# fluhus/frackyfrac

Hardware: NVIDIA B200
Metric: UniFrac sample-pairs/sec (unweighted) (higher is better)
Workload: dtype u8 x u8 -> s32 (tcgen05 kind::i8, exact), s64 chunk / row sums, f32 ratio / output

## Files before the change

### frackyfrac_b200/csrc/frc_internal.h

```cpp
#pragma once
#include <cuda_runtime.h>
#include <cstdint>
#include <string>

namespace frc {

constexpr int kTile = 128;
constexpr int kKBlock = 64;

inline int64_t round_up(int64_t x, int64_t m) { return (x + m - 1) / m * m; }
inline int64_t tri(int64_t i) { return i * (i - 1) / 2; }

struct DevTree {
  int32_t n_nodes = 0;
  int32_t height = 0;
  const int32_t* parent = nullptr;
  const double* length = nullptr;
  const int32_t* child_ptr = nullptr;
  const int32_t* child_idx = nullptr;
  const int32_t* level_nodes = nullptr;
  const int32_t* level_parent = nullptr;
};

struct DevCsr {
  int64_t n_samples = 0;
  int64_t nnz = 0;
  const int64_t* row_ptr = nullptr;
  const int32_t* col = nullptr;
  const double* val = nullptr;
};

struct PeerPtrs {
  uint32_t* p[8] = {nullptr, nullptr, nullptr, nullptr, nullptr, nullptr, nullptr, nullptr};
  int n = 0;
  int self = 0;
};

struct Tile { int32_t ti, tj; };

struct Exceptions {
  unsigned long long* count = nullptr;
  int64_t* index = nullptr;
  double* value = nullptr;
  int32_t cap = 0;
};

int launch_embed_f64(const DevTree& t, const int32_t* level_ptr_host, const DevCsr& a, double* E,
                     int64_t ld, int64_t s_base, cudaStream_t s, int32_t* K = nullptr, int32_t kp = 0);
int launch_totals_f64(const double* E, int32_t n_nodes, int64_t ld, int64_t n_samples,
                      double* total, cudaStream_t s);
int launch_totals_fast_f64(const double* E, int32_t n_nodes, int64_t ld, const double* mult, double* total,
                           double* scratch, cudaStream_t s);
int launch_normalize_f64(double* E, int32_t n_nodes, int64_t ld, int64_t n_samples,
// ... 74 lines not shown
  const double* scale = nullptr;
  const int32_t* shift = nullptr;
  int32_t n = 0;
  bool biased = false;
};
TcOperands* tc_operands_create(const void* P, const void* Bh, const void* Bl, int64_t np, int32_t kp,
                               bool i8, const TcChunks& chunks, const double* len_col, const double* flag_u,
                               std::string* err);
TcOperands* tc_operands_create_bits(const uint32_t* bitsS, int64_t np, int32_t kp, const uint8_t* qa,
                                    const uint8_t* qh, const uint8_t* ql, const TcChunks& chunks,
                                    const double* len_col, const double* flag_u, const long long* r_int,
                                    double unit, std::string* err);
void tc_operands_set_int(TcOperands* o, const long long* r_int, double unit);
void tc_operands_destroy(TcOperands* o);
int tc_chunk_kblocks();
int launch_unweighted_tc(const TcOperands* ops, const double* r, const Tile* tiles, int32_t n_tiles,
                         int64_t n_samples, int64_t first, float* out, double flag_below,
                         uint32_t* flagged, unsigned long long* n_flagged, int num_sms, cudaStream_t s);
int launch_unweighted_fixup(const TcOperands* ops, const uint32_t* flagged,
                            const unsigned long long* n_flagged, unsigned long long* count_host,
                            int64_t first, float* out, const Exceptions& ex, int num_sms, cudaStream_t s);
bool tc_setup(std::string* err);

}
```

### frackyfrac_b200/csrc/job.cu

```cuda
#include <algorithm>
#include <atomic>
#include <chrono>
#include <climits>
#include <cmath>
#include <cstdio>
#include <cstdlib>
#include <cstring>
#include <functional>
#include <memory>
#include <string>
#include <thread>
#include <vector>

#if defined(__x86_64__)
#include <immintrin.h>
#endif

#include "../../include/frcfrc_cuda.h"
#include "frc_internal.h"
#include "host_pool.h"
#include "plan.h"

using namespace frc;
using frc_host::Pool;
// ... 60 lines not shown
constexpr int kMaxParts = 8;

struct Knobs {
  bool trace = false;
  int bands_per_rank = 0;
  int widen_threads = 0;
  int ws_slab = 0;
  bool uw_bf16 = false;
  bool u8_acc_f64 = false;
  bool feed_bits = false;
  bool embed_levels = false;
  int peer_push = -1;
  int group_binades = 3;
  int shard = -1;
  int capacity = -1;
  static Knobs read() {
    Knobs k;
    auto num = [](const char* name, int dflt) { const char* e = getenv(name); return e && *e ? atoi(e) : dflt; };
    auto is = [](const char* name, const char* v) { const char* e = getenv(name); return e && !strcmp(e, v); };
    k.trace = getenv("FRC_TRACE") != nullptr;
    k.bands_per_rank = std::max(0, num("FRC_BANDS", 0));
    k.widen_threads = std::max(0, num("FRC_WIDEN_THREADS", 0));
    k.ws_slab = std::max(0, num("FRC_WS_SLAB", 0));
    k.uw_bf16 = is("FRC_UW_KERNEL", "bf16");
    k.u8_acc_f64 = is("FRC_U8_ACC", "f64");
    k.feed_bits = is("FRC_UW_FEED", "bits");
    k.embed_levels = num("FRC_EMBED_LEVELS", 0) == 1;
    k.peer_push = num("FRC_PEER_PUSH", -1);
    k.group_binades = num("FRC_U8_GROUP_BINADES", 3);
    k.shard = num("FRC_SHARD", -1);
    k.capacity = num("FRC_CAPACITY", -1);
    return k;
  }
};

struct DeviceGuard {
  int prev = -1;
  DeviceGuard() { if (cudaGetDevice(&prev) != cudaSuccess) { prev = -1; cudaGetLastError(); } }
  ~DeviceGuard() { if (prev >= 0) cudaSetDevice(prev); }
};

}

struct DevCtx {
  int device = 0;
  int num_sms = 0;
// ... 68 lines not shown
namespace {

struct Part {
  frc_job* job = nullptr;
  const Shared* sh = nullptr;
  DevCtx* dc = nullptr;
  int index = 0;
  int owner = 0;
  int rc = FRC_OK;
  std::string err;
  frc_info_t info{};

  std::vector<int> mine;
  std::vector<Band> bands;
  std::vector<Tile> tiles;

  int32_t shard_w0 = 0, shard_nw = 0;
  int64_t csr_k0 = 0, csr_k1 = 0;
  PanelMap pm;
  struct CapGroup {
    int shard = 0;
    int64_t first = 0, count = 0;
    int32_t tile_off = 0;
    std::vector<int32_t> coff;
    float* out = nullptr;
    uint32_t* flagged = nullptr;
    unsigned long long* cnt = nullptr;
    unsigned long long* n_flagged_host = nullptr;
    Exceptions ex;
    cudaEvent_t done = nullptr;
// ... 11 lines not shown
  Tile* d_tiles = nullptr;
  int32_t* d_level_ptr = nullptr;
  int32_t* d_post = nullptr;
  unsigned long long* d_flag_counts = nullptr;
  int64_t ws_slab = 0;
  bool peer_push = false;
  uint32_t* d_bits2[2] = {nullptr, nullptr};
  PeerPtrs peers[2];
  int64_t run_count = 0;
  void *d_q0 = nullptr, *d_q1 = nullptr, *d_q2 = nullptr;
  int32_t *d_order = nullptr, *d_col_exp = nullptr;
  uint32_t* d_qam = nullptr;
  uint32_t* d_bitsS = nullptr;
  long long* d_r_int = nullptr;
  long long* d_fix_ws[2] = {nullptr, nullptr};
  uint8_t* d_need = nullptr;
  double *d_lenq = nullptr, *d_len_col = nullptr, *d_flag_u = nullptr, *d_qerr = nullptr;
  TcChunks d_chunks;
  float* d_lenf = nullptr;
  const double* d_mult = nullptr;
  double *d_E = nullptr, *d_total = nullptr, *d_W = nullptr, *d_r = nullptr, *d_scratch = nullptr;
  float* d_A = nullptr;
  int32_t* d_K = nullptr;
  uint32_t *d_bits = nullptr, *d_node_scratch = nullptr;
  void *d_P = nullptr, *d_Bh = nullptr, *d_Bl = nullptr;
  TcOperands* tc = nullptr;
  int64_t* d_list_ptr = nullptr;
  int32_t* d_list_id = nullptr;
  double* d_list_val = nullptr;
  int64_t list_cap = 0;
// ... 356 lines not shown
    else
      launches += launch_exact_pairs(p->d_E, p->dtree.length, sh.B, sh.np, sh.weighted, b.first, b.count, sl.dev64, s);
    PART_CUDA(p, cudaEventRecord(sl.k1, s));
  } else {
    unsigned long long* cnt = p->d_flag_counts + idx;
    *sl.ex.count = 0;
    if (sh.weighted) {
      launches += launch_weighted_tiles(p->pm, sh.np, sh.kp, p->d_lenf, sh.prescale, p->d_W, p->d_tiles + b.tile_off,
                                        b.n_tiles, sh.N, b.first, sl.dev32, kFlagBelowW, sl.flagged, cnt, dc->num_sms, s,
                                        p->d_K);
      PART_CUDA(p, cudaEventRecord(sl.k1, s));
      launches += launch_weighted_fixup(p->dcsr, p->dtree, sh.opts.normalize == 1 ? p->d_total : nullptr, p->d_W,
                                        sl.flagged, cnt, sl.n_flagged_host, b.first, p->d_fix_ws[si], kFixupCtas,
                                        sl.dev32, sl.ex, s, p->d_K, sh.kp);
    } else {
      launches += launch_unweighted_tc(p->tc, p->d_r, p->d_tiles + b.tile_off, b.n_tiles, sh.N, b.first, sl.dev32,
                                       kFlagBelow, sl.flagged, cnt, dc->num_sms, s);
      PART_CUDA(p, cudaEventRecord(sl.k1, s));
      launches += launch_unweighted_fixup(p->tc, sl.flagged, cnt, sl.n_flagged_host, b.first, sl.dev32, sl.ex,
                                          dc->num_sms, s);
    }
  }
  PART_CUDA(p, cudaGetLastError());
  PART_CUDA(p, cudaEventRecord(sl.k2, s));
  if (sh.d2h) {
    cudaStream_t cs = dc->stream[2];
    PART_CUDA(p, cudaStreamWaitEvent(cs, sl.k2, 0));
    if (sh.exact) {
      PART_CUDA(p, cudaMemcpyAsync(sl.host64, sl.dev64, sizeof(double) * b.count, cudaMemcpyDeviceToHost, cs));
      p->info.d2h_bytes += static_cast<int64_t>(sizeof(double)) * b.count;
    } else {
      PART_CUDA(p, cudaMemcpyAsync(sl.host32, sl.dev32, sizeof(float) * b.count, cudaMemcpyDeviceToHost, cs));
// ... 474 lines not shown
      p->max_band = std::max(p->max_band, sh.bands[k].count);
    }
  const bool fast_uw = !sh.exact && !sh.weighted;
  if (sh.capacity) {
    const std::vector<CapGroupPlan> groups =
        plan_capacity_groups(p->bands, sh.N, sh.shards.shard_rows, sh.shards.n_shards, p->tiles, p->band_group);
    for (const CapGroupPlan& gp : groups) {
      if (gp.count >= (1LL << 32)) return pfail(p, FRC_ERR_UNSUPPORTED, "capacity mode: a row shard holds 2^32 pairs or more");
      Part::CapGroup g;
      g.shard = gp.shard; g.first = gp.first; g.count = gp.count; g.tile_off = gp.tile_off; g.coff = gp.coff;
      p->cap.push_back(g);
    }
  } else if (!sh.exact) {
    for (Band& b : p->bands) append_band_tiles(b, fast_uw, p->tiles);
  }
  std::vector<uint8_t> need;
  if (fast_uw && sh.shards.ranges.size() > 1 && sh.fused_embed) need = operand_need_blocks(p->tiles, sh.np, true);
  const Range& own = sh.shards.ranges[p->owner][0];
  p->shard_w0 = static_cast<int32_t>(own.s0 / 32);
  p->shard_nw = static_cast<int32_t>((own.s1 - own.s0) / 32);
  p->csr_k0 = 0; p->csr_k1 = sh.nnz;
  if (sh.exchange != Shared::kNone && fast_uw && sh.N > 0) {
    const int64_t* rp = reinterpret_cast<const int64_t*>(sh.stage_in + sh.in_rowptr.off);
    p->csr_k0 = rp[std::min(sh.N, own.s0)]; p->csr_k1 = rp[std::min(sh.N, own.s1)];
  }
  SegAlloc seg;
  const Seg s_tiles = seg(sizeof(Tile) * p->tiles.size()), s_need = seg(need.size());
  char* st = pin_alloc<char>(p, seg.total);
  if (!st) return p->rc;
  char* d_small = dev_alloc<char>(p, seg.total);
  if (!d_small) return p->rc;
  if (!p->tiles.empty()) memcpy(st + s_tiles.off, p->tiles.data(), s_tiles.bytes);
  if (!need.empty()) memcpy(st + s_need.off, need.data(), s_need.bytes);
  if (!(p->d_plan = dev_alloc<char>(p, sh.plan_bytes))) return p->rc;
  if (!(p->d_in = dev_alloc<char>(p, sh.in_bytes))) return p->rc;
  for (cudaEvent_t* e : {&p->ev_h2d0, &p->ev_h2d1, &p->ev_embed0, &p->ev_embed1, &p->ev_run1})
    PART_CUDA(p, cudaEventCreate(e));
  for (cudaEvent_t* e : {&p->ev_join, &p->ev_bits, &p->ev_rsum, &p->ev_shard})
    PART_CUDA(p, cudaEventCreateWithFlags(e, cudaEventDisableTiming));
  cudaStream_t s0 = dc->stream[0];
  PART_CUDA(p, cudaEventRecord(p->ev_h2d0, s0));
  PART_CUDA(p, cudaMemcpyAsync(p->d_plan, sh.stage_plan, sh.plan_bytes, cudaMemcpyHostToDevice, s0));
  if (seg.total) PART_CUDA(p, cudaMemcpyAsync(d_small, st, seg.total, cudaMemcpyHostToDevice, s0));
  p->info.h2d_bytes = static_cast<int64_t>(sh.plan_bytes + seg.total);
  char* d = p->d_plan;
  char* di = p->d_in;
  p->dcsr.n_samples = sh.N; p->dcsr.nnz = sh.nnz;
  p->dcsr.row_ptr = reinterpret_cast<int64_t*>(di + sh.in_rowptr.off);
// ... 12 lines not shown
  p->d_mult = sh.node_mult ? reinterpret_cast<const double*>(di + sh.in_mult.off) : nullptr;
  p->d_q0 = d + sh.pl_q0.off;
  p->d_q1 = d + sh.pl_hi.off;
  p->d_q2 = d + sh.pl_lo.off;
  p->d_lenq = reinterpret_cast<double*>(d + sh.pl_lenq.off);
  p->d_order = reinterpret_cast<int32_t*>(d + sh.pl_order.off);
  p->d_col_exp = reinterpret_cast<int32_t*>(d + sh.pl_cexp.off);
  p->d_len_col = reinterpret_cast<double*>(d + sh.pl_lcol.off);
  p->d_chunks.end = reinterpret_cast<int32_t*>(d + sh.pl_cend.off);
  p->d_chunks.scale = reinterpret_cast<double*>(d + sh.pl_cscale.off);
  p->d_chunks.n = static_cast<int32_t>(sh.cols.chunk_end.size());
  p->d_chunks.shift = sh.cols.chunk_shift.empty() ? nullptr : reinterpret_cast<int32_t*>(d + sh.pl_cshift.off);
  p->d_chunks.biased = sh.cols.i8 && sh.cols.biased;
  p->d_tiles = reinterpret_cast<Tile*>(d_small + s_tiles.off);
  p->d_need = need.empty() ? nullptr : reinterpret_cast<uint8_t*>(d_small + s_need.off);

  const int chunks = weighted_scratch_chunks(B);
  const bool i8 = sh.cols.i8, intacc = sh.cols.intacc;
  if (sh.exact || sh.weighted) {
    const int64_t per = static_cast<int64_t>(p->shard_nw) * 32;
    p->ws_slab = sh.exact ? sh.np : std::min<int64_t>(per, std::max<int64_t>(kTile, (2LL << 30) / (8LL * B) / kTile * kTile));
    if (!sh.exact && sh.knobs.ws_slab > 0)
      p->ws_slab = std::min<int64_t>(per, round_up(sh.knobs.ws_slab, kTile));
    if (!(p->d_E = dev_alloc<double>(p, static_cast<size_t>(B) * p->ws_slab))) return p->rc;
    if (!(p->d_total = dev_alloc<double>(p, sh.np))) return p->rc;
    if (sh.unsorted_l && !(p->d_list_ptr = dev_alloc<int64_t>(p, sh.N + 2))) return p->rc;
    if (!sh.exact) {
      const size_t a_samples = sh.capacity ? static_cast<size_t>(2 * sh.shards.shard_rows) : static_cast<size_t>(sh.np);
      if (!(p->d_A = dev_alloc<float>(p, static_cast<size_t>(sh.kp) * a_samples))) return p->rc;
      if (sh.keyed && !(p->d_K = dev_alloc<int32_t>(p, static_cast<size_t>(sh.kp) * a_samples))) return p->rc;
// ... 62 lines not shown
    } else if (!(p->d_bits = dev_alloc<uint32_t>(p, std::max<size_t>(words, 64)))) return p->rc;
    const size_t ns = sh.fused_embed ? static_cast<size_t>(presence_node_scratch_words(B, p->shard_nw)) : 0;
    if (ns && !(p->d_node_scratch = dev_alloc<uint32_t>(p, ns))) return p->rc;
    const size_t opsz = sh.bits_feed ? 256 : static_cast<size_t>(sh.np) * sh.kp * (i8 ? 1 : 2);
    if (!(p->d_P = dev_alloc<char>(p, opsz))) return p->rc;
    if (!(p->d_Bh = dev_alloc<char>(p, opsz))) return p->rc;
    if (!(p->d_Bl = dev_alloc<char>(p, opsz))) return p->rc;
    if (sh.bits_feed && !(p->d_bitsS = dev_alloc<uint32_t>(p, static_cast<size_t>(sh.np) * (sh.kp / 32)))) return p->rc;
    if (!(p->d_r = dev_alloc<double>(p, sh.np))) return p->rc;
    if (!(p->d_scratch = dev_alloc<double>(p, static_cast<size_t>(chunks) * sh.np))) return p->rc;
    if (!(p->d_flag_counts = dev_alloc<unsigned long long>(p, p->mine.size() + 1))) return p->rc;
    if (i8 && !(p->d_flag_u = dev_alloc<double>(p, 1))) return p->rc;
    if (i8 && !(p->d_qerr = dev_alloc<double>(p, sh.kp))) return p->rc;
    if (i8 && !(p->d_qam = dev_alloc<uint32_t>(p, sh.kp))) return p->rc;
    if (intacc && !(p->d_r_int = dev_alloc<long long>(p, sh.np))) return p->rc;
    std::string terr;
    if (sh.bits_feed) {
      p->tc = tc_operands_create_bits(p->d_bitsS, sh.np, sh.kp, static_cast<const uint8_t*>(p->d_q0),
                                      static_cast<const uint8_t*>(p->d_q1), static_cast<const uint8_t*>(p->d_q2),
                                      p->d_chunks, p->d_len_col, p->d_flag_u, p->d_r_int,
                                      std::ldexp(1.0, sh.cols.e_min), &terr);
    } else {
      p->tc = tc_operands_create(p->d_P, p->d_Bh, p->d_Bl, sh.np, sh.kp, i8, p->d_chunks, p->d_len_col, p->d_flag_u, &terr);
      if (p->tc && intacc) tc_operands_set_int(p->tc, p->d_r_int, std::ldexp(1.0, sh.cols.e_min));
    }
    if (!p->tc) return pfail(p, FRC_ERR_CUDA, terr);
    if (i8) {
      p->info.kernel_launches += launch_quantize_lengths(
          p->d_len_col, p->d_col_exp, sh.kp, static_cast<uint8_t*>(p->d_q0), static_cast<uint8_t*>(p->d_q1),
          static_cast<uint8_t*>(p->d_q2), p->d_qam, p->d_lenq, p->d_qerr, p->d_flag_u, s0);
// ... 577 lines not shown
```

### frackyfrac_b200/csrc/plan.cpp

```cpp
#include "plan.h"

#include <algorithm>
#include <climits>
#include <cmath>
#include <cstring>

namespace frc {

static std::vector<int> band_owners_lpt(const std::vector<int64_t>& rows, int world) {
  const size_t n = rows.size() > 0 ? rows.size() - 1 : 0;
  std::vector<int> owner(n, 0);
  std::vector<size_t> order(n);
  std::vector<int64_t> cnt(n);
  for (size_t k = 0; k < n; ++k) {
    order[k] = k;
    cnt[k] = tri(rows[k + 1]) - (rows[k] >= 2 ? tri(rows[k]) : 0);
  }
  std::stable_sort(order.begin(), order.end(), [&](size_t a, size_t b) { return cnt[a] > cnt[b]; });
  std::vector<int64_t> load(world, 0);
  for (size_t k : order) {
    int best = 0;
    for (int r = 1; r < world; ++r)
      if (load[r] < load[best]) best = r;
    owner[k] = best;
// ... 256 lines not shown
    const int32_t rows_blk = std::min<int32_t>(9, t1 - t0 + 1);
    const int32_t cols_blk = std::max<int32_t>(1, 74 / rows_blk);
    for (int32_t tb = t0; tb <= t1; tb += rows_blk) {
      const int32_t te = std::min(t1, tb + rows_blk - 1);
      for (int32_t pb = 0; 2 * pb <= te; pb += cols_blk)
        for (int32_t tp = pb; tp < pb + cols_blk && 2 * tp <= te; ++tp)
          for (int32_t ti = std::max(2 * tp, tb); ti <= te; ++ti) tiles.push_back({ti, 2 * tp});
    }
  } else {
    for (int32_t tj = 0; tj <= t1; ++tj)
      for (int32_t ti = std::max(tj, t0); ti <= t1; ++ti) tiles.push_back({ti, tj});
  }
  b.n_tiles = static_cast<int32_t>(tiles.size()) - b.tile_off;
}

std::vector<uint8_t> operand_need_blocks(const std::vector<Tile>& tiles, int64_t np, bool pair_tiles) {
  std::vector<uint8_t> need(static_cast<size_t>((np + 255) / 256), 0);
  const int32_t pairw = pair_tiles ? 2 : 1;
  for (const Tile& t : tiles) {
    need[t.ti / 2] |= 2;
    for (int32_t c = 0; c < pairw; ++c)
      if ((static_cast<int64_t>(t.tj) + c) * kTile < np) need[(t.tj + c) / 2] |= 1;
  }
  return need;
}

bool check_preorder(const int32_t* parent, int32_t B, int32_t* depth, int32_t* bad_parent, int32_t* bad_order) {
  *bad_parent = 0; *bad_order = 0;
  std::vector<int32_t> on_path(B + 1, 0);
  depth[0] = 0;
// ... 138 lines not shown
    for (int c = 0; c <= sp.n_shards; ++c) out_coff[k * (sp.n_shards + 1) + c] = g[k].coff[c];
  }
  for (size_t k = 0; k < tiles.size(); ++k) { out_tiles[2 * k] = tiles[k].ti; out_tiles[2 * k + 1] = tiles[k].tj; }
  return static_cast<int64_t>(g.size());
}

int64_t frc_debug_band_tiles(int64_t row0, int64_t row1, int32_t pair_tiles, int32_t* out2, int64_t cap) {
  frc::Band b;
  b.row0 = row0; b.row1 = row1;
  std::vector<frc::Tile> tiles;
  frc::append_band_tiles(b, pair_tiles != 0, tiles);
  for (size_t k = 0; k < tiles.size() && static_cast<int64_t>(k) < cap; ++k) { out2[2 * k] = tiles[k].ti; out2[2 * k + 1] = tiles[k].tj; }
  return static_cast<int64_t>(tiles.size());
}

int32_t frc_debug_plan_columns(const double* length, int32_t n_nodes, int32_t want_i8, int32_t group_binades,
                               int32_t force_f64, int32_t* col_order, int32_t* col_exp, double* len_col, int32_t cap,
                               int32_t* chunk_end, double* chunk_scale, int32_t* chunk_shift, int32_t* info) {
  const frc::ColumnPlan p = frc::plan_columns(length, n_nodes, want_i8 != 0, group_binades, force_f64 != 0, 64);
  if (p.kp > cap || p.chunk_end.size() > 64) return -p.kp;
  for (int32_t k = 0; k < p.kp; ++k) {
    col_order[k] = p.col_order[k];
    col_exp[k] = p.col_exp.empty() ? 0 : p.col_exp[k];
    len_col[k] = p.len_col[k];
  }
  for (size_t c = 0; c < p.chunk_end.size(); ++c) {
    chunk_end[c] = p.chunk_end[c];
    chunk_scale[c] = p.chunk_scale[c];
    chunk_shift[c] = p.chunk_shift.empty() ? 0 : p.chunk_shift[c];
  }
// ... 28 lines not shown
```

### frackyfrac_b200/csrc/plan.h

```cpp
#pragma once
#include <cstdint>
#include <string>
#include <vector>

#include "frc_internal.h"

namespace frc {

struct Band {
  int64_t row0 = 0, row1 = 0;
  int64_t first = 0, count = 0;
  int32_t tile_off = 0, n_tiles = 0;
  int owner = 0;
};

std::vector<int64_t> band_boundaries(int64_t N, int64_t requested, int world, bool d2h, int per_rank, int value_bytes);
std::vector<int> band_owners(const std::vector<int64_t>& rows, int world);
std::vector<Band> make_bands(int64_t N, int64_t requested, int world, bool d2h, int per_rank, int value_bytes);

struct Range { int64_t s0, s1, slot; };
struct ShardPlan {
  enum Mode { kWhole, kSharded, kCapacity };
  int64_t np = 0, shard_rows = 0;
  int n_shards = 1;
// ... 18 lines not shown
  bool intacc = false;
  bool biased = false;
  int32_t kp = 0;
  int32_t e_min = 0;
  std::vector<int32_t> col_order;
  std::vector<int32_t> col_exp;
  std::vector<double> len_col;
  std::vector<int32_t> chunk_end;
  std::vector<double> chunk_scale;
  std::vector<int32_t> chunk_shift;
};
ColumnPlan plan_columns(const double* length, int32_t n_nodes, bool want_i8, int group_binades, bool force_f64_acc,
                        int bf16_chunk_kblocks);

void append_band_tiles(Band& b, bool pair_tiles, std::vector<Tile>& tiles);
std::vector<uint8_t> operand_need_blocks(const std::vector<Tile>& tiles, int64_t np, bool pair_tiles);

struct TreeLevels {
  int32_t height = -1;
  int32_t bad_parent = 0, bad_order = 0;
  std::vector<int32_t> level_ptr;
};
bool check_preorder(const int32_t* parent, int32_t n_nodes, int32_t* depth, int32_t* bad_parent, int32_t* bad_order);
TreeLevels tree_levels(const int32_t* parent, int32_t n_nodes, int32_t* level_nodes, int32_t* level_parent);
bool tree_children(const int32_t* parent, int32_t n_nodes, int32_t* child_ptr, int32_t* child_idx);
void tree_post_order(const int32_t* parent, int32_t n_nodes, int32_t* post_order);

struct PrunedTree {
  int32_t n_nodes = 0;
  std::vector<int32_t> parent, new_of_old;
// ... 7 lines not shown
```

### frackyfrac_b200/csrc/unweighted_tc.cu

```cuda
#include <cuda.h>
#include <cuda_runtime.h>

#include <cstdio>
#include <cstdlib>
#include <type_traits>

#include "frc_internal.h"
#include "ptx.cuh"
#include "wire.cuh"

namespace frc {

namespace {

constexpr int BM = 128, BN = 128, BK = 64, UK = 16;
constexpr int A_BYTES = BM * BK * 2;
constexpr int B_BYTES = BN * BK * 2;
constexpr int EPI_WARP0 = 2;
constexpr int DN = 2 * BN;
constexpr uint32_t TMEM_COLS = 2 * DN;

constexpr int STAGES2 = 6;
constexpr int STAGE2_BYTES = A_BYTES + B_BYTES;
constexpr int NUM_BARS2 = 2 * STAGES2 + 4;
// ... 57 lines not shown
#pragma unroll
    for (int x = 0; x < 8; ++x) {
      const int64_t i = i0 + n0 + x;
      if (i < n_samples && j < i) {
        out[off] = dv[x];
        if (fu[x]) {
          unsigned long long slot = atomicAdd(n_flagged, 1ULL);
          flagged[slot] = static_cast<uint32_t>(off);
        }
      }
      off += i;
    }
  }
}

template <int kMode>
__global__ void __cluster_dims__(2, 1, 1) __launch_bounds__(THREADS2, 1)
k_unweighted_tc2(const __grid_constant__ CUtensorMap mapP, const __grid_constant__ CUtensorMap mapBh,
                 const __grid_constant__ CUtensorMap mapBl, const int32_t* __restrict__ chunk_end,
                 const double* __restrict__ chunk_scale, const int32_t* __restrict__ chunk_shift,
                 int32_t n_chunks, int32_t biased, const double* __restrict__ r,
                 const long long* __restrict__ r_int, double unit, const Tile* __restrict__ tiles, int32_t n_tiles,
                 int64_t n_samples, int64_t first, float* __restrict__ out, double flag_below,
                 const double* __restrict__ flag_u_ptr, uint32_t* __restrict__ flagged,
                 unsigned long long* __restrict__ n_flagged, int dbg) {
  (void)dbg;
  constexpr bool kI8 = kMode != 0;
  constexpr bool kInt = kMode == 2;
  extern __shared__ uint8_t smem_raw[];
  const uint32_t raw = ptx::smem_u32(smem_raw);
  const uint32_t pad = ((raw + 1023u) & ~1023u) - raw;
  uint8_t* smem = smem_raw + pad;
  const uint32_t smem_base = raw + pad;
  const uint32_t bar_base = smem_base + STAGES2 * STAGE2_BYTES;
  auto full_bar = [&](int s) { return bar_base + 8u * s; };
  auto empty_bar = [&](int s) { return bar_base + 8u * (STAGES2 + s); };
  auto tfull_bar = [&](int b) { return bar_base + 8u * (2 * STAGES2 + b); };
  auto tempty_bar = [&](int b) { return bar_base + 8u * (2 * STAGES2 + 2 + b); };
  volatile uint32_t* tmem_slot =
      reinterpret_cast<volatile uint32_t*>(smem + STAGES2 * STAGE2_BYTES + NUM_BARS2 * 8);

  const int warp = threadIdx.x >> 5;
  const int lane = threadIdx.x & 31;
  const uint32_t cta = ptx::cluster_ctarank();
  const int pair = blockIdx.x >> 1;
  const int n_pairs = gridDim.x >> 1;

  if (warp == 0 && lane == 0) {
    ptx::prefetch_tensormap(&mapP);
    ptx::prefetch_tensormap(cta == 0 ? &mapBh : &mapBl);
    for (int s = 0; s < STAGES2; ++s) {
      ptx::mbar_init(full_bar(s), 1);
      ptx::mbar_init(empty_bar(s), 1);
    }
    for (int b = 0; b < 2; ++b) {
      ptx::mbar_init(tfull_bar(b), 1);
      ptx::mbar_init(tempty_bar(b), 2 * EPI2_WARPS);
    }
    ptx::fence_barrier_init();
    ptx::fence_proxy_async();
  }
  if (warp == 1) {
    ptx::tmem_alloc<2>(ptx::smem_u32(const_cast<uint32_t*>(tmem_slot)), TMEM_COLS);
    ptx::tmem_relinquish<2>();
  }
  ptx::tc_fence_before();
  ptx::cluster_sync_all();
  ptx::tc_fence_after();
  const uint32_t tmem_base = *tmem_slot;

  const int n_kblocks = chunk_end[n_chunks - 1];

  if (warp == 0) {
    if (lane == 0) {
      int stage = 0;
      uint32_t phase = 0;
      const void* mapB = cta == 0 ? static_cast<const void*>(&mapBh) : static_cast<const void*>(&mapBl);
      constexpr int kElems = kI8 ? BKB : BKB / 2;
      TL(long long w_empty = 0;)
      for (int t = pair; t < n_tiles; t += n_pairs) {
        const Tile tile = tiles[t];
        const int row_a = (tile.tj + static_cast<int>(cta)) * BM, row_b = tile.ti * BN;
        for (int kb = 0; kb < n_kblocks; ++kb) {
          TL(const long long c0 = clock64();)
          ptx::mbar_wait(empty_bar(stage), phase ^ 1u);
          TL(w_empty += clock64() - c0;)
          const uint32_t sa = smem_base + stage * STAGE2_BYTES;
          if (cta == 0)
            ptx::mbar_expect_tx(full_bar(stage), 2 * ((TL_ON(2) ? 0 : A_BYTES) + (TL_ON(1) ? 0 : B_BYTES)));
          const uint32_t lead_bar = ptx::mapa_u32(full_bar(stage), 0);
          if (!TL_ON(2)) ptx::tma_load_2d_2sm(sa, &mapP, lead_bar, kb * kElems, row_a);
          if (!TL_ON(1)) ptx::tma_load_2d_2sm(sa + A_BYTES, mapB, lead_bar, kb * kElems, row_b);
          if (++stage == STAGES2) { stage = 0; phase ^= 1u; }
        }
      }
      TL(g_tc_dbg[blockIdx.x * 8 + 3] = w_empty;)
    }
    __syncwarp();
  } else if (warp == 1) {
    if (lane == 0 && cta == 0) {
      constexpr uint32_t idesc = kI8 ? ptx::umma_idesc_u8(2 * BM, DN) : ptx::umma_idesc_bf16(2 * BM, DN);
      int stage = 0;
      uint32_t phase = 0;
      uint32_t chunk = 0;
      TL(long long w_tempty = 0; long long w_full = 0; const long long c_start = clock64();)
      for (int t = pair; t < n_tiles; t += n_pairs) {
        int kb = 0;
        for (int ch = 0; ch < n_chunks; ++ch, ++chunk) {
          const uint32_t buf = chunk & 1u;
          TL(const long long c0 = clock64();)
          ptx::mbar_wait(tempty_bar(buf), ((chunk >> 1) & 1u) ^ 1u);
          TL(w_tempty += clock64() - c0;)
          ptx::tc_fence_after();
          const uint32_t d_tmem = tmem_base + buf * DN;
          const int kb_begin = kb, kb_end = chunk_end[ch];
          for (; kb < kb_end; ++kb) {
            TL(const long long c1 = clock64();)
            ptx::mbar_wait(full_bar(stage), phase);
            TL(w_full += clock64() - c1;)
            ptx::tc_fence_after();
            const uint32_t sa = smem_base + stage * STAGE2_BYTES;
            const uint64_t da = ptx::umma_desc_k_sw128(sa);
            const uint64_t db = ptx::umma_desc_k_sw128(sa + A_BYTES);
#pragma unroll
            for (int k = 0; k < 4; ++k) {
              const uint32_t accum = (kb > kb_begin || k > 0) ? 1u : 0u;
              if constexpr (kI8) ptx::umma_i8<2>(d_tmem, da + 2u * k, db + 2u * k, idesc, accum);
              else ptx::umma_bf16<2>(d_tmem, da + 2u * k, db + 2u * k, idesc, accum);
            }
            ptx::umma_commit_2sm(empty_bar(stage), 3);
// ... 1 lines not shown
          }
          ptx::umma_commit_2sm(tfull_bar(buf), 3);
        }
      }
      TL(g_tc_dbg[blockIdx.x * 8 + 0] = w_tempty; g_tc_dbg[blockIdx.x * 8 + 1] = w_full;
         g_tc_dbg[blockIdx.x * 8 + 2] = clock64() - c_start;)
    }
    __syncwarp();
  } else {
    const int q = warp & 3;
    const int cg = (warp - EPI_WARP0) >> 2;
    using Acc = typename std::conditional<kInt, unsigned long long,
                                          typename std::conditional<kI8, double, float>::type>::type;
    const float flag_u = flag_u_ptr ? static_cast<float>(*flag_u_ptr) : 0.f;
    const float flag_d = static_cast<float>(flag_below);
    const long long flag_u_int = (kInt && flag_u_ptr) ? static_cast<long long>(*flag_u_ptr / unit) : 0;
    double acc0 = 0.0;
    if constexpr (kI8 && !kInt)
      if (biased) for (int ch = 0; ch < n_chunks; ++ch) acc0 -= 4503599627370496.0 * chunk_scale[ch];
    uint32_t chunk = 0;
    TL(long long w_tfull = 0; long long t_drain = 0; long long t_ratio = 0; const long long e_start = clock64();)
    for (int t = pair; t < n_tiles; t += n_pairs) {
      const Tile tile = tiles[t];
      Acc acc[EPI2_COLS];
#pragma unroll
      for (int n = 0; n < EPI2_COLS; ++n) acc[n] = static_cast<Acc>(acc0);
      for (int ch = 0; ch < n_chunks; ++ch, ++chunk) {
        const uint32_t buf = chunk & 1u;
        const double scale = (kI8 && !kInt) ? chunk_scale[ch] : 1.0;
        const uint32_t shift = kInt ? static_cast<uint32_t>(chunk_shift[ch]) : 0u;
        TL(const long long c0 = clock64();)
        ptx::mbar_wait(tfull_bar(buf), (chunk >> 1) & 1u);
        TL(const long long c1 = clock64();)
        ptx::tc_fence_after();
        const uint32_t taddr = tmem_base + (static_cast<uint32_t>(q * 32) << 16) + buf * DN + cg * EPI2_COLS;
        if constexpr (kInt) {
          drain_int(taddr, shift, acc);
        } else if constexpr (kI8) {
          auto drain = [&](auto kBiased) {
            uint32_t v[2][8], w[2][8];
            ptx::tmem_ld_32x8(taddr, v[0]);
            ptx::tmem_ld_32x8(taddr + BN, w[0]);
// ... 19 lines not shown
          for (int cc = 0; cc < EPI2_COLS / 16; ++cc) {
            uint32_t v[16], w[16];
            ptx::tmem_ld_32x16(taddr + cc * 16, v);
            ptx::tmem_ld_32x16(taddr + BN + cc * 16, w);
            ptx::tmem_ld_wait();
#pragma unroll
            for (int x = 0; x < 16; ++x) acc[cc * 16 + x] += __uint_as_float(v[x]) + __uint_as_float(w[x]);
          }
        }
        ptx::tc_fence_before();
        __syncwarp();
        if (lane == 0) ptx::mbar_arrive_cluster(tempty_bar(buf), 0);
        TL(w_tfull += c1 - c0; t_drain += clock64() - c1;)
      }
      TL(const long long c2 = clock64();)
      const int64_t j = static_cast<int64_t>(tile.tj + static_cast<int>(cta)) * BM + q * 32 + lane;
      const int64_t i0 = static_cast<int64_t>(tile.ti) * BN + cg * EPI2_COLS;
      static_assert(EPI2_COLS == 32, "r[i] is broadcast from lane n");
      if (TL_ON(4)) {
        if (acc[0] == static_cast<Acc>(-1.5)) out[0] = 0.f;
      } else if (static_cast<int64_t>(tile.tj + static_cast<int>(cta)) * BM + q * 32 < i0 + EPI2_COLS) {
        int64_t off = i0 * (i0 - 1) / 2 - first + j;
        if constexpr (kInt) {
          ratio_int(acc, r_int, i0, j, lane, n_samples, off, flag_u_int, out, flagged, n_flagged);
        } else {
          const double rj = j < n_samples ? r[j] : 0.0;
          const double ri_lane = r[i0 + lane];
#pragma unroll
          for (int n0 = 0; n0 < EPI2_COLS; n0 += 8) {
            float dv[8], uv[8];
#pragma unroll
            for (int x = 0; x < 8; ++x) {
              const double ri = __shfl_sync(0xffffffffu, ri_lane, n0 + x);
              const double sd = static_cast<double>(acc[n0 + x]);
              const double U = fma(-2.0, sd, ri + rj);
              uv[x] = static_cast<float>(U);
              dv[x] = __fdividef(uv[x], uv[x] + static_cast<float>(sd));
            }
#pragma unroll
// ... 468 lines not shown
  if (clear) { static unsigned long long z[512 * 8] = {0}; cudaMemcpyToSymbol(frc::g_bits_dbg, z, sizeof(z)); }
  return rc;
#else
  (void)out; (void)n; (void)clear;
  return -1;
#endif
}
namespace frc {

int tc_chunk_kblocks() {
  const char* e = getenv("FRC_TC_CHUNK_KBLOCKS");
  int x = e ? atoi(e) : 64;
  return x < 1 ? 1 : x;
}

int launch_unweighted_tc(const TcOperands* ops, const double* r, const Tile* tiles, int32_t n_tiles,
                         int64_t n_samples, int64_t first, float* out, double flag_below,
                         uint32_t* flagged, unsigned long long* n_flagged, int num_sms, cudaStream_t s) {
  if (n_tiles <= 0) return 0;
  const int pairs = num_sms / 2;
  const int grid = 2 * (n_tiles < pairs ? n_tiles : pairs);
  const TcChunks& c = ops->chunks;
  if (ops->from_bits) {
    k_unweighted_bits2<<<grid, bits::THREADS, bits::SMEM_BYTES, s>>>(
        ops->mapBits, ops->qa, ops->qh, ops->ql, c.end, c.shift, c.n, ops->r_int, ops->unit, tiles, n_tiles, n_samples,
        first, out, ops->flag_u, flagged, n_flagged);
    return 1;
  }
#define FRC_TC2_ARGS ops->mapP, ops->mapBh, ops->mapBl, c.end, c.scale, c.shift, c.n, c.biased ? 1 : 0, r, ops->r_int, \
                     ops->unit, tiles, n_tiles, n_samples, first, out, flag_below, ops->flag_u, flagged, n_flagged, ops->dbg
  if (ops->i8 && ops->r_int) k_unweighted_tc2<2><<<grid, THREADS2, SMEM2_BYTES, s>>>(FRC_TC2_ARGS);
  else if (ops->i8) k_unweighted_tc2<1><<<grid, THREADS2, SMEM2_BYTES, s>>>(FRC_TC2_ARGS);
  else k_unweighted_tc2<0><<<grid, THREADS2, SMEM2_BYTES, s>>>(FRC_TC2_ARGS);
#undef FRC_TC2_ARGS
  return 1;
}

int launch_unweighted_fixup(const TcOperands* ops, const uint32_t* flagged, const unsigned long long* n_flagged,
                            unsigned long long* count_host, int64_t first, float* out, const Exceptions& ex,
                            int num_sms, cudaStream_t s) {
  const auto kernel = ops->from_bits ? k_unweighted_fixup<Rows::kBits>
                      : ops->i8      ? k_unweighted_fixup<Rows::kU8>
                                     : k_unweighted_fixup<Rows::kBf16>;
  const void* rows = ops->from_bits ? static_cast<const void*>(ops->bitsS) : ops->P;
  kernel<<<num_sms * 4, 256, 0, s>>>(rows, ops->kp, ops->len_col, flagged, n_flagged, count_host, first, out, ex);
// ... 5 lines not shown
```

Baseline: 30.89 billion.

## Split tail tiles across idle CTA pairs along K with split-K reduction

Replaces the round-robin tile loop in the unweighted tcgen05 kernel with a host-planned per-pair work list. When the tile count is not a multiple of the number of CTA pairs, the leftover tiles are split along the K dimension into up to three pieces spread over idle pairs. The partial integer accumulators are combined through a global workspace with an atomic counter, and the last piece to arrive runs the ratio epilogue. This targets the wave-quantization tail where most SMs sit idle during the last round of tiles. In exchange it adds global-memory partial writes and reads, threadfence and atomic synchronization, and extra planning and allocation.

```diff
diff --git a/frackyfrac_b200/csrc/frc_internal.h b/frackyfrac_b200/csrc/frc_internal.h
--- a/frackyfrac_b200/csrc/frc_internal.h
+++ b/frackyfrac_b200/csrc/frc_internal.h
@@ -37,6 +37,10 @@
 };
 
 struct Tile { int32_t ti, tj; };
+
+struct PairUnit { int32_t tile, kb0, kb1, piece, n_pieces, slot; };
+constexpr int kMaxPieces = 3;
+constexpr int kMinPieceKb = 8;
 
 struct Exceptions {
   unsigned long long* count = nullptr;
@@ -141,8 +145,17 @@
 void tc_operands_set_int(TcOperands* o, const long long* r_int, double unit);
 void tc_operands_destroy(TcOperands* o);
 int tc_chunk_kblocks();
+struct PairWork {
+  const PairUnit* units = nullptr;
+  const int32_t* ptr = nullptr;
+  int32_t busy = 0;
+  unsigned long long* ws = nullptr;
+  uint32_t* cnt = nullptr;
+};
+size_t tc_split_ws_words(int32_t n_slots);
+size_t tc_split_cnt_words(int32_t n_slots);
 int launch_unweighted_tc(const TcOperands* ops, const double* r, const Tile* tiles, int32_t n_tiles,
-                         int64_t n_samples, int64_t first, float* out, double flag_below,
+                         const PairWork& work, int64_t n_samples, int64_t first, float* out, double flag_below,
                          uint32_t* flagged, unsigned long long* n_flagged, int num_sms, cudaStream_t s);
 int launch_unweighted_fixup(const TcOperands* ops, const uint32_t* flagged,
                             const unsigned long long* n_flagged, unsigned long long* count_host,
diff --git a/frackyfrac_b200/csrc/job.cu b/frackyfrac_b200/csrc/job.cu
--- a/frackyfrac_b200/csrc/job.cu
+++ b/frackyfrac_b200/csrc/job.cu
@@ -98,6 +98,7 @@
   int group_binades = 3;
   int shard = -1;
   int capacity = -1;
+  bool uw_split = true;
   static Knobs read() {
     Knobs k;
     auto num = [](const char* name, int dflt) { const char* e = getenv(name); return e && *e ? atoi(e) : dflt; };
@@ -114,6 +115,7 @@
     k.group_binades = num("FRC_U8_GROUP_BINADES", 3);
     k.shard = num("FRC_SHARD", -1);
     k.capacity = num("FRC_CAPACITY", -1);
+    k.uw_split = num("FRC_UW_SPLIT", 1) != 0;
     return k;
   }
 };
@@ -212,6 +214,10 @@
   std::vector<int> mine;
   std::vector<Band> bands;
   std::vector<Tile> tiles;
+  struct BandWork { int32_t ptr_off = 0, busy = 0; };
+  std::vector<BandWork> band_work;
+  std::vector<PairUnit> units;
+  std::vector<int32_t> unit_ptr;
 
   int32_t shard_w0 = 0, shard_nw = 0;
   int64_t csr_k0 = 0, csr_k1 = 0;
@@ -253,6 +259,10 @@
   uint32_t* d_bitsS = nullptr;
   long long* d_r_int = nullptr;
   long long* d_fix_ws[2] = {nullptr, nullptr};
+  PairUnit* d_units = nullptr;
+  int32_t* d_unit_ptr = nullptr;
+  unsigned long long* d_split_ws[2] = {nullptr, nullptr};
+  uint32_t* d_split_cnt[2] = {nullptr, nullptr};
   uint8_t* d_need = nullptr;
   double *d_lenq = nullptr, *d_len_col = nullptr, *d_flag_u = nullptr, *d_qerr = nullptr;
   TcChunks d_chunks;
@@ -639,8 +649,14 @@
                                         sl.flagged, cnt, sl.n_flagged_host, b.first, p->d_fix_ws[si], kFixupCtas,
                                         sl.dev32, sl.ex, s, p->d_K, sh.kp);
     } else {
-      launches += launch_unweighted_tc(p->tc, p->d_r, p->d_tiles + b.tile_off, b.n_tiles, sh.N, b.first, sl.dev32,
-                                       kFlagBelow, sl.flagged, cnt, dc->num_sms, s);
+      PairWork work;
+      if (!p->band_work.empty()) {
+        const Part::BandWork& bw = p->band_work[idx];
+        work.units = p->d_units; work.ptr = p->d_unit_ptr + bw.ptr_off; work.busy = bw.busy;
+        work.ws = p->d_split_ws[si]; work.cnt = p->d_split_cnt[si];
+      }
+      launches += launch_unweighted_tc(p->tc, p->d_r, p->d_tiles + b.tile_off, b.n_tiles, work, sh.N, b.first,
+                                       sl.dev32, kFlagBelow, sl.flagged, cnt, dc->num_sms, s);
       PART_CUDA(p, cudaEventRecord(sl.k1, s));
       launches += launch_unweighted_fixup(p->tc, sl.flagged, cnt, sl.n_flagged_host, b.first, sl.dev32, sl.ex,
                                           dc->num_sms, s);
@@ -1145,6 +1161,18 @@
   } else if (!sh.exact) {
     for (Band& b : p->bands) append_band_tiles(b, fast_uw, p->tiles);
   }
+  int32_t split_slots = 0;
+  if (fast_uw && !sh.bits_feed) {
+    const bool split = sh.cols.i8 && sh.cols.intacc && sh.knobs.uw_split;
+    for (const Band& b : p->bands) {
+      const PairSchedule ps = plan_pair_schedule(b.n_tiles, dc->num_sms / 2, sh.cols.chunk_end.back(), split);
+      p->band_work.push_back({static_cast<int32_t>(p->unit_ptr.size()), ps.busy});
+      const int32_t base = static_cast<int32_t>(p->units.size());
+      for (int32_t v : ps.ptr) p->unit_ptr.push_back(base + v);
+      p->units.insert(p->units.end(), ps.units.begin(), ps.units.end());
+      split_slots = std::max(split_slots, ps.n_slots);
+    }
+  }
   std::vector<uint8_t> need;
   if (fast_uw && sh.shards.ranges.size() > 1 && sh.fused_embed) need = operand_need_blocks(p->tiles, sh.np, true);
   const Range& own = sh.shards.ranges[p->owner][0];
@@ -1157,12 +1185,15 @@
   }
   SegAlloc seg;
   const Seg s_tiles = seg(sizeof(Tile) * p->tiles.size()), s_need = seg(need.size());
+  const Seg s_units = seg(sizeof(PairUnit) * p->units.size()), s_uptr = seg(sizeof(int32_t) * p->unit_ptr.size());
   char* st = pin_alloc<char>(p, seg.total);
   if (!st) return p->rc;
   char* d_small = dev_alloc<char>(p, seg.total);
   if (!d_small) return p->rc;
   if (!p->tiles.empty()) memcpy(st + s_tiles.off, p->tiles.data(), s_tiles.bytes);
   if (!need.empty()) memcpy(st + s_need.off, need.data(), s_need.bytes);
+  if (!p->units.empty()) memcpy(st + s_units.off, p->units.data(), s_units.bytes);
+  if (!p->unit_ptr.empty()) memcpy(st + s_uptr.off, p->unit_ptr.data(), s_uptr.bytes);
   if (!(p->d_plan = dev_alloc<char>(p, sh.plan_bytes))) return p->rc;
   if (!(p->d_in = dev_alloc<char>(p, sh.in_bytes))) return p->rc;
   for (cudaEvent_t* e : {&p->ev_h2d0, &p->ev_h2d1, &p->ev_embed0, &p->ev_embed1, &p->ev_run1})
@@ -1205,6 +1236,8 @@
   p->d_chunks.biased = sh.cols.i8 && sh.cols.biased;
   p->d_tiles = reinterpret_cast<Tile*>(d_small + s_tiles.off);
   p->d_need = need.empty() ? nullptr : reinterpret_cast<uint8_t*>(d_small + s_need.off);
+  p->d_units = reinterpret_cast<PairUnit*>(d_small + s_units.off);
+  p->d_unit_ptr = reinterpret_cast<int32_t*>(d_small + s_uptr.off);
 
   const int chunks = weighted_scratch_chunks(B);
   const bool i8 = sh.cols.i8, intacc = sh.cols.intacc;
@@ -1297,6 +1330,12 @@
     if (i8 && !(p->d_qerr = dev_alloc<double>(p, sh.kp))) return p->rc;
     if (i8 && !(p->d_qam = dev_alloc<uint32_t>(p, sh.kp))) return p->rc;
     if (intacc && !(p->d_r_int = dev_alloc<long long>(p, sh.np))) return p->rc;
+    if (split_slots > 0)
+      for (int k = 0; k < 2; ++k) {
+        if (!(p->d_split_ws[k] = dev_alloc<unsigned long long>(p, tc_split_ws_words(split_slots)))) return p->rc;
+        if (!(p->d_split_cnt[k] = dev_alloc<uint32_t>(p, tc_split_cnt_words(split_slots)))) return p->rc;
+        PART_CUDA(p, cudaMemsetAsync(p->d_split_cnt[k], 0, sizeof(uint32_t) * tc_split_cnt_words(split_slots), s0));
+      }
     std::string terr;
     if (sh.bits_feed) {
       p->tc = tc_operands_create_bits(p->d_bitsS, sh.np, sh.kp, static_cast<const uint8_t*>(p->d_q0),
diff --git a/frackyfrac_b200/csrc/plan.cpp b/frackyfrac_b200/csrc/plan.cpp
--- a/frackyfrac_b200/csrc/plan.cpp
+++ b/frackyfrac_b200/csrc/plan.cpp
@@ -294,6 +294,43 @@
   b.n_tiles = static_cast<int32_t>(tiles.size()) - b.tile_off;
 }
 
+PairSchedule plan_pair_schedule(int32_t n_tiles, int32_t n_pairs, int32_t n_kblocks, bool split) {
+  PairSchedule s;
+  std::vector<std::vector<PairUnit>> per(n_pairs);
+  const int32_t R = n_tiles % n_pairs;
+  const int32_t G = n_kblocks / kMinPieceKb;
+  const int32_t whole = split && R > 0 && G >= 2 ? n_tiles - R : n_tiles;
+  for (int32_t t = 0; t < whole; ++t) per[t % n_pairs].push_back({t, 0, n_kblocks, 0, 1, -1});
+  if (whole < n_tiles) {
+    const int64_t total = static_cast<int64_t>(R) * G;
+    const int32_t m = (G + kMaxPieces - 2) / (kMaxPieces - 1);
+    const int32_t used = static_cast<int32_t>(std::min<int64_t>(n_pairs, total / m));
+    std::vector<int32_t> pieces(R, 0);
+    for (int32_t p = 0; p < used; ++p) {
+      const int64_t g0 = total * p / used, g1 = total * (p + 1) / used;
+      for (int32_t r = static_cast<int32_t>(g0 / G); r <= static_cast<int32_t>((g1 - 1) / G); ++r) {
+        const int64_t a = std::max<int64_t>(g0, static_cast<int64_t>(r) * G) - static_cast<int64_t>(r) * G;
+        const int64_t b = std::min<int64_t>(g1, static_cast<int64_t>(r + 1) * G) - static_cast<int64_t>(r) * G;
+        per[p].push_back({whole + r, static_cast<int32_t>(a * n_kblocks / G), static_cast<int32_t>(b * n_kblocks / G),
+                          pieces[r]++, 0, -1});
+      }
+    }
+    std::vector<int32_t> slot(R, -1);
+    for (int32_t r = 0; r < R; ++r)
+      if (pieces[r] > 1) slot[r] = s.n_slots++;
+    for (int32_t p = 0; p < used; ++p)
+      for (PairUnit& u : per[p])
+        if (u.tile >= whole) { u.n_pieces = pieces[u.tile - whole]; u.slot = slot[u.tile - whole]; }
+  }
+  s.ptr.assign(n_pairs + 1, 0);
+  for (int32_t p = 0; p < n_pairs; ++p) {
+    s.units.insert(s.units.end(), per[p].begin(), per[p].end());
+    s.ptr[p + 1] = static_cast<int32_t>(s.units.size());
+    if (!per[p].empty()) s.busy = p + 1;
+  }
+  return s;
+}
+
 std::vector<uint8_t> operand_need_blocks(const std::vector<Tile>& tiles, int64_t np, bool pair_tiles) {
   std::vector<uint8_t> need(static_cast<size_t>((np + 255) / 256), 0);
   const int32_t pairw = pair_tiles ? 2 : 1;
@@ -462,6 +499,19 @@
   return static_cast<int64_t>(tiles.size());
 }
 
+int64_t frc_debug_pair_schedule(int32_t n_tiles, int32_t n_pairs, int32_t n_kblocks, int32_t split, int32_t* ptr,
+                                int32_t* out6, int64_t cap, int32_t* info) {
+  const frc::PairSchedule s = frc::plan_pair_schedule(n_tiles, n_pairs, n_kblocks, split != 0);
+  for (size_t p = 0; p < s.ptr.size(); ++p) ptr[p] = s.ptr[p];
+  for (size_t k = 0; k < s.units.size() && static_cast<int64_t>(k) < cap; ++k) {
+    const frc::PairUnit& u = s.units[k];
+    const int32_t v[6] = {u.tile, u.kb0, u.kb1, u.piece, u.n_pieces, u.slot};
+    for (int c = 0; c < 6; ++c) out6[6 * k + c] = v[c];
+  }
+  info[0] = s.busy; info[1] = s.n_slots;
+  return static_cast<int64_t>(s.units.size());
+}
+
 int32_t frc_debug_plan_columns(const double* length, int32_t n_nodes, int32_t want_i8, int32_t group_binades,
                                int32_t force_f64, int32_t* col_order, int32_t* col_exp, double* len_col, int32_t cap,
                                int32_t* chunk_end, double* chunk_scale, int32_t* chunk_shift, int32_t* info) {
diff --git a/frackyfrac_b200/csrc/plan.h b/frackyfrac_b200/csrc/plan.h
--- a/frackyfrac_b200/csrc/plan.h
+++ b/frackyfrac_b200/csrc/plan.h
@@ -56,6 +56,14 @@
                         int bf16_chunk_kblocks);
 
 void append_band_tiles(Band& b, bool pair_tiles, std::vector<Tile>& tiles);
+
+struct PairSchedule {
+  std::vector<int32_t> ptr;
+  std::vector<PairUnit> units;
+  int32_t busy = 0;
+  int32_t n_slots = 0;
+};
+PairSchedule plan_pair_schedule(int32_t n_tiles, int32_t n_pairs, int32_t n_kblocks, bool split);
 std::vector<uint8_t> operand_need_blocks(const std::vector<Tile>& tiles, int64_t np, bool pair_tiles);
 
 struct TreeLevels {
diff --git a/frackyfrac_b200/csrc/unweighted_tc.cu b/frackyfrac_b200/csrc/unweighted_tc.cu
--- a/frackyfrac_b200/csrc/unweighted_tc.cu
+++ b/frackyfrac_b200/csrc/unweighted_tc.cu
@@ -95,13 +95,42 @@
   }
 }
 
+constexpr size_t kSplitWarpWords = 32 * EPI2_COLS;
+__device__ __forceinline__ bool add_pieces(unsigned long long (&acc)[EPI2_COLS], const PairUnit& w, uint32_t cta, int we,
+                                           int lane, unsigned long long* __restrict__ ws, uint32_t* __restrict__ cnt) {
+  auto part = [&](int piece) {
+    return ws + ((((static_cast<size_t>(w.slot) * kMaxPieces + piece) * 2 + cta) * EPI2_WARPS + we) * kSplitWarpWords) + lane;
+  };
+  unsigned long long* mine = part(w.piece);
+#pragma unroll
+  for (int x = 0; x < EPI2_COLS; ++x) mine[32 * x] = acc[x];
+  __threadfence();
+  __syncwarp();
+  uint32_t* c = cnt + (static_cast<size_t>(w.slot) * 2 + cta) * EPI2_WARPS + we;
+  uint32_t seen = 0;
+  if (lane == 0) seen = atomicAdd(c, 1u);
+  seen = __shfl_sync(0xffffffffu, seen, 0);
+  if (static_cast<int>(seen) != w.n_pieces - 1) return false;
+  __threadfence();
+  for (int p = 0; p < w.n_pieces; ++p) {
+    if (p == w.piece) continue;
+    const unsigned long long* other = part(p);
+#pragma unroll
+    for (int x = 0; x < EPI2_COLS; ++x) acc[x] += __ldcg(other + 32 * x);
+  }
+  if (lane == 0) *c = 0;
+  return true;
+}
+
 template <int kMode>
 __global__ void __cluster_dims__(2, 1, 1) __launch_bounds__(THREADS2, 1)
 k_unweighted_tc2(const __grid_constant__ CUtensorMap mapP, const __grid_constant__ CUtensorMap mapBh,
                  const __grid_constant__ CUtensorMap mapBl, const int32_t* __restrict__ chunk_end,
                  const double* __restrict__ chunk_scale, const int32_t* __restrict__ chunk_shift,
                  int32_t n_chunks, int32_t biased, const double* __restrict__ r,
-                 const long long* __restrict__ r_int, double unit, const Tile* __restrict__ tiles, int32_t n_tiles,
+                 const long long* __restrict__ r_int, double unit, const Tile* __restrict__ tiles,
+                 const PairUnit* __restrict__ units, const int32_t* __restrict__ unit_ptr,
+                 unsigned long long* __restrict__ split_ws, uint32_t* __restrict__ split_cnt,
                  int64_t n_samples, int64_t first, float* __restrict__ out, double flag_below,
                  const double* __restrict__ flag_u_ptr, uint32_t* __restrict__ flagged,
                  unsigned long long* __restrict__ n_flagged, int dbg) {
@@ -125,7 +154,6 @@
   const int lane = threadIdx.x & 31;
   const uint32_t cta = ptx::cluster_ctarank();
   const int pair = blockIdx.x >> 1;
-  const int n_pairs = gridDim.x >> 1;
 
   if (warp == 0 && lane == 0) {
     ptx::prefetch_tensormap(&mapP);
@@ -149,8 +177,6 @@
   ptx::cluster_sync_all();
   ptx::tc_fence_after();
   const uint32_t tmem_base = *tmem_slot;
-
-  const int n_kblocks = chunk_end[n_chunks - 1];
 
   if (warp == 0) {
     if (lane == 0) {
@@ -159,10 +185,11 @@
       const void* mapB = cta == 0 ? static_cast<const void*>(&mapBh) : static_cast<const void*>(&mapBl);
       constexpr int kElems = kI8 ? BKB : BKB / 2;
       TL(long long w_empty = 0;)
-      for (int t = pair; t < n_tiles; t += n_pairs) {
-        const Tile tile = tiles[t];
+      for (int u = unit_ptr[pair], u_end = unit_ptr[pair + 1]; u < u_end; ++u) {
+        const PairUnit w = units[u];
+        const Tile tile = tiles[w.tile];
         const int row_a = (tile.tj + static_cast<int>(cta)) * BM, row_b = tile.ti * BN;
-        for (int kb = 0; kb < n_kblocks; ++kb) {
+        for (int kb = w.kb0; kb < w.kb1; ++kb) {
           TL(const long long c0 = clock64();)
           ptx::mbar_wait(empty_bar(stage), phase ^ 1u);
           TL(w_empty += clock64() - c0;)
@@ -185,16 +212,18 @@
       uint32_t phase = 0;
       uint32_t chunk = 0;
       TL(long long w_tempty = 0; long long w_full = 0; const long long c_start = clock64();)
-      for (int t = pair; t < n_tiles; t += n_pairs) {
-        int kb = 0;
-        for (int ch = 0; ch < n_chunks; ++ch, ++chunk) {
+      for (int u = unit_ptr[pair], u_end = unit_ptr[pair + 1]; u < u_end; ++u) {
+        const PairUnit w = units[u];
+        int ch = 0;
+        while (chunk_end[ch] <= w.kb0) ++ch;
+        for (int kb = w.kb0; kb < w.kb1; ++ch, ++chunk) {
           const uint32_t buf = chunk & 1u;
           TL(const long long c0 = clock64();)
           ptx::mbar_wait(tempty_bar(buf), ((chunk >> 1) & 1u) ^ 1u);
           TL(w_tempty += clock64() - c0;)
           ptx::tc_fence_after();
           const uint32_t d_tmem = tmem_base + buf * DN;
-          const int kb_begin = kb, kb_end = chunk_end[ch];
+          const int kb_begin = kb, kb_end = min(chunk_end[ch], w.kb1);
           for (; kb < kb_end; ++kb) {
             TL(const long long c1 = clock64();)
             ptx::mbar_wait(full_bar(stage), phase);
@@ -226,18 +255,19 @@
                                           typename std::conditional<kI8, double, float>::type>::type;
     const float flag_u = flag_u_ptr ? static_cast<float>(*flag_u_ptr) : 0.f;
     const float flag_d = static_cast<float>(flag_below);
-    const long long flag_u_int = (kInt && flag_u_ptr) ? static_cast<long long>(*flag_u_ptr / unit) : 0;
     double acc0 = 0.0;
     if constexpr (kI8 && !kInt)
       if (biased) for (int ch = 0; ch < n_chunks; ++ch) acc0 -= 4503599627370496.0 * chunk_scale[ch];
     uint32_t chunk = 0;
     TL(long long w_tfull = 0; long long t_drain = 0; long long t_ratio = 0; const long long e_start = clock64();)
-    for (int t = pair; t < n_tiles; t += n_pairs) {
-      const Tile tile = tiles[t];
+    for (int u = unit_ptr[pair], u_end = unit_ptr[pair + 1]; u < u_end; ++u) {
+      const int kb0 = units[u].kb0, kb1 = units[u].kb1;
       Acc acc[EPI2_COLS];
 #pragma unroll
       for (int n = 0; n < EPI2_COLS; ++n) acc[n] = static_cast<Acc>(acc0);
-      for (int ch = 0; ch < n_chunks; ++ch, ++chunk) {
+      int ch = 0;
+      while (chunk_end[ch] <= kb0) ++ch;
+      for (int kb = kb0; kb < kb1; kb = chunk_end[ch++], ++chunk) {
         const uint32_t buf = chunk & 1u;
         const double scale = (kI8 && !kInt) ? chunk_scale[ch] : 1.0;
         const uint32_t shift = kInt ? static_cast<uint32_t>(chunk_shift[ch]) : 0u;
@@ -287,6 +317,8 @@
         TL(w_tfull += c1 - c0; t_drain += clock64() - c1;)
       }
       TL(const long long c2 = clock64();)
+      const PairUnit pu = units[u];
+      const Tile tile = tiles[pu.tile];
       const int64_t j = static_cast<int64_t>(tile.tj + static_cast<int>(cta)) * BM + q * 32 + lane;
       const int64_t i0 = static_cast<int64_t>(tile.ti) * BN + cg * EPI2_COLS;
       static_assert(EPI2_COLS == 32, "r[i] is broadcast from lane n");
@@ -295,7 +327,10 @@
       } else if (static_cast<int64_t>(tile.tj + static_cast<int>(cta)) * BM + q * 32 < i0 + EPI2_COLS) {
         int64_t off = i0 * (i0 - 1) / 2 - first + j;
         if constexpr (kInt) {
-          ratio_int(acc, r_int, i0, j, lane, n_samples, off, flag_u_int, out, flagged, n_flagged);
+          if (pu.n_pieces == 1 || add_pieces(acc, pu, cta, warp - EPI_WARP0, lane, split_ws, split_cnt)) {
+            const long long flag_u_int = flag_u_ptr ? static_cast<long long>(*flag_u_ptr / unit) : 0;
+            ratio_int(acc, r_int, i0, j, lane, n_samples, off, flag_u_int, out, flagged, n_flagged);
+          }
         } else {
           const double rj = j < n_samples ? r[j] : 0.0;
           const double ri_lane = r[i0 + lane];
@@ -794,21 +829,28 @@
   return x < 1 ? 1 : x;
 }
 
+size_t tc_split_ws_words(int32_t n_slots) {
+  return static_cast<size_t>(n_slots) * kMaxPieces * 2 * EPI2_WARPS * kSplitWarpWords;
+}
+size_t tc_split_cnt_words(int32_t n_slots) { return static_cast<size_t>(n_slots) * 2 * EPI2_WARPS; }
+
 int launch_unweighted_tc(const TcOperands* ops, const double* r, const Tile* tiles, int32_t n_tiles,
-                         int64_t n_samples, int64_t first, float* out, double flag_below,
+                         const PairWork& work, int64_t n_samples, int64_t first, float* out, double flag_below,
                          uint32_t* flagged, unsigned long long* n_flagged, int num_sms, cudaStream_t s) {
   if (n_tiles <= 0) return 0;
-  const int pairs = num_sms / 2;
-  const int grid = 2 * (n_tiles < pairs ? n_tiles : pairs);
   const TcChunks& c = ops->chunks;
   if (ops->from_bits) {
+    const int pairs = num_sms / 2;
+    const int grid = 2 * (n_tiles < pairs ? n_tiles : pairs);
     k_unweighted_bits2<<<grid, bits::THREADS, bits::SMEM_BYTES, s>>>(
         ops->mapBits, ops->qa, ops->qh, ops->ql, c.end, c.shift, c.n, ops->r_int, ops->unit, tiles, n_tiles, n_samples,
         first, out, ops->flag_u, flagged, n_flagged);
     return 1;
   }
+  const int grid = 2 * work.busy;
 #define FRC_TC2_ARGS ops->mapP, ops->mapBh, ops->mapBl, c.end, c.scale, c.shift, c.n, c.biased ? 1 : 0, r, ops->r_int, \
-                     ops->unit, tiles, n_tiles, n_samples, first, out, flag_below, ops->flag_u, flagged, n_flagged, ops->dbg
+                     ops->unit, tiles, work.units, work.ptr, work.ws, work.cnt, n_samples, first, out, flag_below,      \
+                     ops->flag_u, flagged, n_flagged, ops->dbg
   if (ops->i8 && ops->r_int) k_unweighted_tc2<2><<<grid, THREADS2, SMEM2_BYTES, s>>>(FRC_TC2_ARGS);
   else if (ops->i8) k_unweighted_tc2<1><<<grid, THREADS2, SMEM2_BYTES, s>>>(FRC_TC2_ARGS);
   else k_unweighted_tc2<0><<<grid, THREADS2, SMEM2_BYTES, s>>>(FRC_TC2_ARGS);
```

Result: slower. 30.30 billion (median of 6 runs) (-1.9%).
